# GuoleiSun/VSS-CFFM

Measured on AMD Instinct MI355X. Metric: clips/sec (fwd+bwd) CFFM-B1 480x480 T=4 hot path (CFFA+CFM, decoder_focal depth 2), higher is better.
Workload: dtype f32 in/out, f32 accumulate; MFMA operands: split-bf16 (hi+lo, ~2^-17) in the Linear GEMMs, f16 in QK^T/AV

## Files before the change

vss_cffm_amd/csrc/panel_kernels.h:

```cpp
#pragma once
#include "cffm_common.h"
#include "gemm_kernels.h"
#include "dws_kernels.h"

#define PNL_KC 256
#define PNL_THREADS 512
#define PNL_WAVES 8
__device__ __forceinline__ int pnl_off(int row, int chunk) { return row * PNL_KC + (((chunk ^ row) & 15) << 3) + ((chunk & 16) << 3); }
#define PNL_IMG(MT) (16 * (MT) * PNL_KC)
#define PNL_LDS(MT) (2 * 2 * PNL_IMG(MT) * 2 + 2 * PNL_THREADS * 16)

__device__ __host__ __forceinline__ long pnl_frag_unit(int jt, int ks, int h, int KS) { return ((long)(jt * KS + ks) * 2 + h) * 64; }

__device__ __forceinline__ void pnl_pack_weight(const float* __restrict__ W, int N, int K, bool nn, f32x4* __restrict__ dst, long item) {
    const int lane = (int)(item & 63);
    const long u = item >> 6;
    const int OUT = nn ? K : N, KS = (nn ? N : K) / 32;
    const int ks = (int)(u % KS), jt = (int)(u / KS);
    if (jt * 16 >= OUT) return;
    const int l15 = lane & 15, g = lane >> 4;
    bf16x8 hi, lo;
#pragma unroll
    for (int e = 0; e < 8; ++e) {
        const int o = 16 * jt + l15, c = 32 * ks + 8 * g + e;
        const float x = nn ? W[(long)c * K + o] : W[(long)o * K + c];
        hi[e] = (bf16)x;
        lo[e] = (bf16)(x - (float)hi[e]);
    }
    dst[pnl_frag_unit(jt, ks, 0, KS) + lane] = __builtin_bit_cast(f32x4, hi);
    dst[pnl_frag_unit(jt, ks, 1, KS) + lane] = __builtin_bit_cast(f32x4, lo);
}
__global__ void __launch_bounds__(256) k_pnl_pack_weight(const float* __restrict__ W, int N, int K, int nn, f32x4* __restrict__ dst) {
    const long item = (long)blockIdx.x * 256 + threadIdx.x;
    if (item < (long)N * K / 8) pnl_pack_weight(W, N, K, nn != 0, dst, item);
}

struct PnlPackJobs { const float* w[4]; f32x4* dst[4]; int N[4], K[4]; long end[4]; int n, nn; };
__global__ void __launch_bounds__(256) k_pnl_pack_weights(PnlPackJobs J) {
    long item = (long)blockIdx.x * 256 + threadIdx.x;
    int j = 0;
#pragma unroll
    for (int q = 0; q < 3; ++q)
        if (q + 1 < J.n && item >= J.end[q]) j = q + 1;
    if (j > 0) item -= J.end[j - 1];
    if (item < (long)J.N[j] * J.K[j] / 8) pnl_pack_weight(J.w[j], J.N[j], J.K[j], J.nn != 0, J.dst[j], item);
}

__device__ __forceinline__ void pnl_lds_barrier() {
#ifdef CFFM_EMU
    __syncthreads();
#else
    __builtin_amdgcn_fence(__ATOMIC_RELEASE, "workgroup", "local");
    __builtin_amdgcn_s_barrier();
    __builtin_amdgcn_fence(__ATOMIC_ACQUIRE, "workgroup", "local");
#endif
}

template <int MT>
struct PnlStage { f32x4 v[2 * MT]; };
template <int MT>
__device__ __forceinline__ void pnl_stage_load(PnlStage<MT>& r, buf_t rs, int lda, int m0, int kc0, int tid) {
#pragma unroll
    for (int it = 0; it < 2 * MT; ++it) {
        const int item = tid + PNL_THREADS * it, row = item >> 6, c4 = item & 63;
        r.v[it] = buf_ld16(rs, (uint32_t)((row * lda + 4 * c4) * 4), (uint32_t)(((long)m0 * lda + kc0) * 4));
    }
}
template <int MT, bool PRE>
__device__ __forceinline__ void pnl_stage_store(const PnlStage<MT>& r, bf16* __restrict__ hi, bf16* __restrict__ lo, int tid) {
#pragma unroll
    for (int it = 0; it < 2 * MT; ++it) {
        const int item = tid + PNL_THREADS * it, row = item >> 6, c4 = item & 63;
        bf16x4 h, l;
        if (PRE) unsplit4(r.v[it], h, l);
        else split4(r.v[it], h, l);
        const int o = pnl_off(row, c4 >> 1) + 4 * (c4 & 1);
        *(bf16x4*)(hi + o) = h;
        *(bf16x4*)(lo + o) = l;
    }
}

template <int NT, int D>
struct PnlRing { f32x4 v[D][NT][2]; };

struct PnlStream {
    buf_t rs;
    uint32_t voff;
    int KS;
};
template <int NT, int D>
__device__ __forceinline__ void pnl_ring_load(PnlRing<NT, D>& ring, int slot, const PnlStream& st, int jt, int ks) {
#pragma unroll
    for (int j = 0; j < NT; ++j)
#pragma unroll
        for (int h = 0; h < 2; ++h)
            ring.v[slot][j][h] = buf_ld16(st.rs, st.voff, (uint32_t)(pnl_frag_unit(jt + j, ks, h, st.KS) * 16));
}

__device__ __forceinline__ void pnl_pin_vmem() {
#ifndef CFFM_EMU
    __builtin_amdgcn_sched_barrier(0);
#endif
}
struct PnlNoExtra { __device__ __forceinline__ void operator()(int) const {} };
template <int MT, int NTW, int NT, int D, class Extra = PnlNoExtra, bool LAST = false>
__device__ __forceinline__ void pnl_chunk_mma(f32x4 (&acc)[NTW][MT], PnlRing<NT, D>& ring, const bf16* __restrict__ Ahi,
                                              const bf16* __restrict__ Alo, const PnlStream& st, int jt0, int ks0, int l15, int g,
                                              const PnlStream& nst, int njt0, int nks0, const Extra& extra = Extra()) {
    constexpr int NPASS = NTW / NT, SC = NPASS * 8;
    static_assert(NTW % NT == 0 && SC % D == 0 && D <= SC && D >= 2, "ring depth must divide the steps of a chunk");
    bf16x8 ah[2][MT], al[2][MT];
#pragma unroll
    for (int i = 0; i < MT; ++i) {
        ah[0][i] = *(const bf16x8*)(Ahi + pnl_off(16 * i + l15, g));
        al[0][i] = *(const bf16x8*)(Alo + pnl_off(16 * i + l15, g));
    }
#pragma unroll
    for (int sc = 0; sc < SC; ++sc) {
        const int p = sc / 8, cur = sc & 1;
        const int sn = sc + D - 1, slot_n = sn % D;
        if (sn < SC) pnl_ring_load<NT, D>(ring, slot_n, st, jt0 + (sn / 8) * NT, ks0 + sn % 8);
        else if (!LAST) pnl_ring_load<NT, D>(ring, slot_n, nst, njt0 + ((sn - SC) / 8) * NT, nks0 + (sn - SC) % 8);
        extra(sc);
        pnl_pin_vmem();
        if (sc + 1 < SC) {
            const int k8n = (sc + 1) % 8;
#pragma unroll
            for (int i = 0; i < MT; ++i) {
                ah[cur ^ 1][i] = *(const bf16x8*)(Ahi + pnl_off(16 * i + l15, 4 * k8n + g));
                al[cur ^ 1][i] = *(const bf16x8*)(Alo + pnl_off(16 * i + l15, 4 * k8n + g));
            }
        }
        const int slot = sc % D;
#pragma unroll
        for (int j = 0; j < NT; ++j) {
            const bf16x8 bh = __builtin_bit_cast(bf16x8, ring.v[slot][j][0]), bl = __builtin_bit_cast(bf16x8, ring.v[slot][j][1]);
#pragma unroll
            for (int i = 0; i < MT; ++i) {
                f32x4 c = acc[p * NT + j][i];
                c = mfma16x16x32_bf16(bh, al[cur][i], c);
                c = mfma16x16x32_bf16(bl, ah[cur][i], c);
                c = mfma16x16x32_bf16(bh, ah[cur][i], c);
                acc[p * NT + j][i] = c;
            }
        }
    }
}

template <int MT>
__device__ __forceinline__ void pnl_tfrag_store(const bf16* __restrict__ hi, const bf16* __restrict__ lo, f32x4* __restrict__ dst, int m0, int jt0, int CT,
                                                long R, long R32, int wave, int lane) {
    const int l15 = lane & 15, g = lane >> 4;
    constexpr int NRG = 2 * MT, NOP = (NRG + 3) / 4;
#pragma unroll
    for (int q = 0; q < 32 * NOP / PNL_WAVES; ++q) {
        const int item = wave + PNL_WAVES * q;
        const int u = item / NOP, op = item % NOP, jt = u >> 1, h = u & 1;
        const int rgl = 4 * op + g;
        const bf16* img = h ? lo : hi;
        const int row = 8 * (rgl < NRG ? rgl : 0) + (l15 >> 2), col = 16 * jt + 4 * (l15 & 3);
        const bf16x4 a = lds_tr4_bf16(img + pnl_off(row, col >> 3) + (col & 4));
        const bf16x4 b = lds_tr4_bf16(img + pnl_off(row + 4, col >> 3) + (col & 4));
        const long rg = (long)(m0 >> 3) + rgl, r0 = 8 * rg;
        bf16x8 f;
#pragma unroll
        for (int e = 0; e < 4; ++e) {
            f[e] = r0 + e < R ? a[e] : (bf16)0.f;
            f[4 + e] = r0 + 4 + e < R ? b[e] : (bf16)0.f;
        }
        const bool tail = (NRG % 4 != 0) && rgl >= NRG && (long)m0 + 16 * MT >= R;
        if ((rgl < NRG || tail) && r0 < R32) dst[tfrag_unit(rg >> 2, jt0 + jt, h, CT) + 16 * (int)(rg & 3) + l15] = __builtin_bit_cast(f32x4, f);
    }
}

__device__ __forceinline__ uint32_t pnl_l2_touch(const void* w, long bytes, int tid) {
    const long nlines = bytes >> 7;
    const int nsl = (int)(gridDim.x >> 3) > 0 ? (int)(gridDim.x >> 3) : 1, rank = (int)(blockIdx.x >> 3) % nsl;
    const long per = (nlines + nsl - 1) / nsl, l = rank * per + tid;
    return (tid < per && l < nlines) ? *(const uint32_t*)((const char*)w + (l << 7)) : 0u;
}
template <int MT, int NTW, int NT, int D, bool A_PRE, int EPI>
__global__ void __launch_bounds__(PNL_THREADS) k_panel_gemm(const float* __restrict__ A, int lda, int M, int K, const f32x4* __restrict__ Wf,
                                                            float* __restrict__ C, int ldc, const float* __restrict__ bias,
                                                            float* __restrict__ colrec = nullptr,
                                                            f32x4* __restrict__ a_t = nullptr ) {
    CFFM_DYN_SMEM(smem);
    bf16* img = (bf16*)smem;
    f32x4* csum = (f32x4*)(img + 4 * PNL_IMG(MT));
#define PNL_COLSUM_PUT(c_)                                                                        \
    if (!A_PRE && colrec) {                                                                       \
        f32x4 s_ = sr.v[0];                                                                       \
        _Pragma("unroll") for (int it = 1; it < 2 * MT; ++it) s_ += sr.v[it];                     \
        csum[((c_) & 1) * PNL_THREADS + tid] = s_;                                                \
    }
#define PNL_COLSUM_GET(c_)                                                                        \
    if (!A_PRE && colrec && wave == ((c_) & 7)) {                                                 \
        const f32x4* p_ = csum + ((c_) & 1) * PNL_THREADS + lane;                                 \
        f32x4 t_ = p_[0];                                                                         \
        _Pragma("unroll") for (int w = 1; w < PNL_WAVES; ++w) t_ += p_[64 * w];                   \
        *(f32x4*)(colrec + (long)blockIdx.x * K + (c_) * PNL_KC + 4 * lane) = t_;                 \
    }
    const int tid = threadIdx.x, lane = tid & 63, wave = wave_uniform(tid >> 6), l15 = lane & 15, g = lane >> 4;
    const int m0 = blockIdx.x * 16 * MT;
    const int NCH = K / PNL_KC, KS = K / 32, N = PNL_WAVES * NTW * 16;
    const buf_t rsa = buf_make(A, (uint32_t)((long)M * lda * 4));
    PnlStream st;
    st.rs = buf_make(Wf, (uint32_t)((long)N * K * 4));
    st.voff = lane * 16;
    st.KS = KS;
    const int jt0 = wave * NTW;
    f32x4 acc[NTW][MT];
#pragma unroll
    for (int t = 0; t < NTW; ++t)
#pragma unroll
        for (int i = 0; i < MT; ++i) acc[t][i] = (f32x4){0.f, 0.f, 0.f, 0.f};
    PnlRing<NT, D> ring;
#pragma unroll
    for (int s = 0; s < D - 1; ++s) pnl_ring_load<NT, D>(ring, s, st, jt0 + (s / 8) * NT, s % 8);
    pnl_pin_vmem();
    PnlStage<MT> sr;
    pnl_stage_load<MT>(sr, rsa, lda, m0, 0, tid);
    pnl_stage_store<MT, A_PRE>(sr, img, img + PNL_IMG(MT), tid);
    PNL_COLSUM_PUT(0)
    if (NCH > 1) pnl_stage_load<MT>(sr, rsa, lda, m0, PNL_KC, tid);
    pnl_lds_barrier();
    for (int c = 0; c < NCH; ++c) {
        PNL_COLSUM_GET(c)
        const bf16* hi = img + (c & 1) * 2 * PNL_IMG(MT);
        pnl_chunk_mma<MT, NTW, NT, D>(acc, ring, hi, hi + PNL_IMG(MT), st, jt0, 8 * c, l15, g, st, jt0, 8 * (c + 1));
        if (a_t) pnl_tfrag_store<MT>(hi, hi + PNL_IMG(MT), a_t, m0, 16 * c, K / 16, M, ((long)M + 31) / 32 * 32, wave, lane);
        if (c + 1 < NCH) {
            bf16* nx = img + ((c + 1) & 1) * 2 * PNL_IMG(MT);
            pnl_stage_store<MT, A_PRE>(sr, nx, nx + PNL_IMG(MT), tid);
            PNL_COLSUM_PUT(c + 1)
            if (c + 2 < NCH) pnl_stage_load<MT>(sr, rsa, lda, m0, (c + 2) * PNL_KC, tid);
            pnl_lds_barrier();
        }
    }
#undef PNL_COLSUM_PUT
#undef PNL_COLSUM_GET
    {
        static_assert(EPI == 0, "k_panel_gemm epilogue");
        constexpr int ESZ = 4, NCOL = PNL_WAVES * NTW * 16, ROWB = NCOL * ESZ + 32, UPR = NCOL * ESZ / 16;
        static_assert(16 * MT * ROWB <= PNL_LDS(MT), "panel output does not fit the image buffers");
        char* out = (char*)smem;
        __syncthreads();
#pragma unroll
        for (int t = 0; t < NTW; ++t) {
            const int n = 16 * (jt0 + t) + 4 * g;
            f32x4 bv = (f32x4){0.f, 0.f, 0.f, 0.f};
            if (bias) bv = *(const f32x4*)(bias + n);
#pragma unroll
            for (int i = 0; i < MT; ++i) {
                *(f32x4*)(out + (16 * i + l15) * ROWB + n * ESZ) = acc[t][i] + bv;
            }
        }
        __syncthreads();
        char* dst = (char*)C;
        for (int u = tid; u < 16 * MT * UPR; u += PNL_THREADS) {
            const int r = u / UPR, c = u % UPR;
            if (m0 + r < M) *(f32x4*)(dst + ((long)(m0 + r) * ldc) * ESZ + 16 * c) = *(const f32x4*)(out + r * ROWB + 16 * c);
        }
    }
}

#define QKV3_LDS(MT) (2 * PNL_IMG(MT) * 2)
template <int MT>
__global__ void __launch_bounds__(PNL_THREADS, 4) k_panel_qkv3(const float* __restrict__ xs, int M, const f32x4* __restrict__ Wf,
                                                               const float* __restrict__ bias, h16* __restrict__ qkv16, f32x4* __restrict__ x_t) {
    constexpr int NTW = 2, D = 2, KS = CFFM_C / 32;
    static_assert(CFFM_C == PNL_KC && PNL_WAVES * NTW * 16 == CFFM_C, "one chunk, 256 columns per third");
    CFFM_DYN_SMEM(smem);
    bf16* img = (bf16*)smem;
    const int tid = threadIdx.x, lane = tid & 63, wave = wave_uniform(tid >> 6), l15 = lane & 15, g = lane >> 4;
    const int q = blockIdx.x >> 3, t = q % 3, pan = 8 * (q / 3) + (blockIdx.x & 7);
    if (pan >= (M + 16 * MT - 1) / (16 * MT)) return;
    const int m0 = pan * 16 * MT;
    const buf_t rsa = buf_make(xs, (uint32_t)((long)M * CFFM_C * 4));
    PnlStream st;
    st.rs = buf_make(Wf, (uint32_t)(3 * CFFM_C * CFFM_C * 4));
    st.voff = lane * 16;
    st.KS = KS;
    const int jt0 = 16 * t + wave * NTW;
    f32x4 acc[NTW][MT];
#pragma unroll
    for (int j = 0; j < NTW; ++j)
#pragma unroll
        for (int i = 0; i < MT; ++i) acc[j][i] = (f32x4){0.f, 0.f, 0.f, 0.f};
    PnlRing<2, D> ring;
    pnl_ring_load<2, D>(ring, 0, st, jt0, 0);
    pnl_pin_vmem();
    {
        PnlStage<MT> sr;
        pnl_stage_load<MT>(sr, rsa, CFFM_C, m0, 0, tid);
        pnl_stage_store<MT, true>(sr, img, img + PNL_IMG(MT), tid);
    }
    pnl_lds_barrier();
    pnl_chunk_mma<MT, NTW, 2, D, PnlNoExtra, true>(acc, ring, img, img + PNL_IMG(MT), st, jt0, 0, l15, g, st, jt0, 0);
    if (x_t && t == 0) pnl_tfrag_store<MT>(img, img + PNL_IMG(MT), x_t, m0, 0, CFFM_C / 16, M, ((long)M + 31) / 32 * 32, wave, lane);
    constexpr int ROWB = CFFM_C * 2 + 32, UPR = CFFM_C * 2 / 16;
    static_assert(16 * MT * ROWB <= QKV3_LDS(MT), "panel output does not fit the image");
    char* out = (char*)smem;
    pnl_lds_barrier();
    const float sc = t == 0 ? 0.17677669529663687f : 1.f;
#pragma unroll
    for (int j = 0; j < NTW; ++j) {
        const int nl = 16 * (wave * NTW + j) + 4 * g;
        const f32x4 bv = *(const f32x4*)(bias + CFFM_C * t + nl);
#pragma unroll
        for (int i = 0; i < MT; ++i) {
            typedef h16 h16x4 __attribute__((ext_vector_type(4)));
            h16x4 o;
            for (int e = 0; e < 4; ++e) o[e] = (h16)((acc[j][i][e] + bv[e]) * sc);
            *(h16x4*)(out + (16 * i + l15) * ROWB + nl * 2) = o;
        }
    }
    pnl_lds_barrier();
    char* dst = (char*)qkv16 + CFFM_C * 2 * t;
    for (int u = tid; u < 16 * MT * UPR; u += PNL_THREADS) {
        const int r = u / UPR, c = u % UPR;
        if (m0 + r < M) *(f32x4*)(dst + (long)(m0 + r) * (3 * CFFM_C * 2) + 16 * c) = *(const f32x4*)(out + r * ROWB + 16 * c);
    }
}

__device__ __forceinline__ f32x4 pnl_pack_hl(bf16x4 h, bf16x4 l) {
    const f32x2_t a = __builtin_bit_cast(f32x2_t, h), b = __builtin_bit_cast(f32x2_t, l);
    return (f32x4){a[0], a[1], b[0], b[1]};
}
__device__ __forceinline__ void pnl_img_put(bf16* __restrict__ hi, bf16* __restrict__ lo, int row, int n, bf16x4 h, bf16x4 l) {
    const int o = pnl_off(row, n >> 3) + (n & 4);
    *(bf16x4*)(hi + o) = h;
    *(bf16x4*)(lo + o) = l;
}
__device__ __forceinline__ float pnl_sum_g(float v) {
    v += __shfl_xor(v, 16, 64);
    v += __shfl_xor(v, 32, 64);
    return v;
}
#define PNL_STORE4(p, v) (*(f32x4*)(p) = (v))
#define PNL_FUSED_LDS(MT) (6 * PNL_IMG(MT) * 2 + 2 * PNL_WAVES * 16 * (MT) * 4)

struct MlpFwdArgs {
    const float* ao;
    const float* xt; long xt_bs; int rows_per_batch;
    const f32x4 *wp, *w1, *w2;
    const float *bp, *b1, *b2, *g2, *be2;
    float *x1, *z2s , *mean2, *rstd2, *hraw, *acts , *x2;
    f32x4 *ao_t, *z2_t, *act_t;
    int NP;
};

template <int MT, int D, bool INFER = false>
__global__ void __launch_bounds__(PNL_THREADS) k_mlp_fwd(MlpFwdArgs a) {
    CFFM_DYN_SMEM(smem);
    bf16* P = (bf16*)smem;
    bf16* ACT = P + 2 * PNL_IMG(MT);
    float* red = (float*)(ACT + 4 * PNL_IMG(MT));
    const int tid = threadIdx.x, lane = tid & 63, wave = wave_uniform(tid >> 6), l15 = lane & 15, g = lane >> 4;
    const int m0 = blockIdx.x * 16 * MT, NP = a.NP;
    PnlStream sp, s1, s2;
    sp.rs = buf_make(a.wp, 256u * 256 * 4); sp.voff = lane * 16; sp.KS = 8;
    s1.rs = buf_make(a.w1, 1024u * 256 * 4); s1.voff = lane * 16; s1.KS = 8;
    s2.rs = buf_make(a.w2, 1024u * 256 * 4); s2.voff = lane * 16; s2.KS = 32;
    PnlRing<2, D> ring;
#pragma unroll
    for (int s = 0; s < D - 1; ++s) pnl_ring_load<2, D>(ring, s, sp, 2 * wave, s);
    uint32_t touch = 0;
    pnl_pin_vmem();
    {
        PnlStage<MT> sr;
        pnl_stage_load<MT>(sr, buf_make(a.ao, (uint32_t)((long)NP * 256 * 4)), 256, m0, 0, tid);
        pnl_pin_vmem();
        const uint32_t t0 = pnl_l2_touch(a.w1, 1024L * 256 * 4, tid), t1 = pnl_l2_touch(a.w2, 1024L * 256 * 4, tid);
        pnl_pin_vmem();
        pnl_stage_store<MT, false>(sr, P, P + PNL_IMG(MT), tid);
        touch = t0 ^ t1;
    }
    pnl_lds_barrier();
    const long NP32 = ((long)NP + 31) / 32 * 32;
    if (!INFER && a.ao_t) pnl_tfrag_store<MT>(P, P + PNL_IMG(MT), a.ao_t, m0, 0, 16, NP, NP32, wave, lane);
    const f32x4 z4 = (f32x4){0.f, 0.f, 0.f, 0.f};
    f32x4 acc[2][MT];
#pragma unroll
    for (int t = 0; t < 2; ++t)
#pragma unroll
        for (int i = 0; i < MT; ++i) acc[t][i] = z4;
    pnl_chunk_mma<MT, 2, 2, D>(acc, ring, P, P + PNL_IMG(MT), sp, 2 * wave, 0, l15, g, s1, 2 * wave, 0);
    f32x4 x1v[2][MT];
    bool valid[MT];
    long mrow[MT];
    float s[MT];
#pragma unroll
    for (int i = 0; i < MT; ++i) {
        const long m = m0 + 16 * i + l15;
        valid[i] = m < NP;
        mrow[i] = m;
        s[i] = 0.f;
    }
#pragma unroll
    for (int t = 0; t < 2; ++t) {
        const int n = 32 * wave + 16 * t + 4 * g;
        const f32x4 bv = *(const f32x4*)(a.bp + n);
#pragma unroll
        for (int i = 0; i < MT; ++i) {
            f32x4 r = z4;
            if (valid[i]) {
                const long b = mrow[i] / a.rows_per_batch, rr = mrow[i] % a.rows_per_batch;
                r = *(const f32x4*)(a.xt + b * a.xt_bs + rr * 256 + n);
            }
            const f32x4 v = acc[t][i] + bv + r;
            x1v[t][i] = v;
            if (!INFER && valid[i]) *(f32x4*)(a.x1 + mrow[i] * 256 + n) = v;
            s[i] += (v[0] + v[1]) + (v[2] + v[3]);
        }
    }
#pragma unroll
    for (int i = 0; i < MT; ++i) {
        s[i] = pnl_sum_g(s[i]);
        if (g == 0) red[wave * 16 * MT + 16 * i + l15] = s[i];
    }
    pnl_lds_barrier();
    float mu[MT], rs[MT];
#pragma unroll
    for (int i = 0; i < MT; ++i) {
        float tot = 0.f;
#pragma unroll
        for (int w = 0; w < PNL_WAVES; ++w) tot += red[w * 16 * MT + 16 * i + l15];
        mu[i] = tot * (1.f / 256);
        float q = 0.f;
#pragma unroll
        for (int t = 0; t < 2; ++t) {
            const f32x4 d = x1v[t][i] - mu[i];
            q += (d[0] * d[0] + d[1] * d[1]) + (d[2] * d[2] + d[3] * d[3]);
        }
        q = pnl_sum_g(q);
        if (g == 0) red[(PNL_WAVES + wave) * 16 * MT + 16 * i + l15] = q;
    }
    pnl_lds_barrier();
#pragma unroll
    for (int i = 0; i < MT; ++i) {
        float tot = 0.f;
#pragma unroll
        for (int w = 0; w < PNL_WAVES; ++w) tot += red[(PNL_WAVES + w) * 16 * MT + 16 * i + l15];
        rs[i] = 1.f / sqrtf(tot * (1.f / 256) + CFFM_LN_EPS);
        if (!INFER && wave == 0 && g == 0 && valid[i]) { a.mean2[mrow[i]] = mu[i]; a.rstd2[mrow[i]] = rs[i]; }
    }
#pragma unroll
    for (int t = 0; t < 2; ++t) {
        const int n = 32 * wave + 16 * t + 4 * g;
        const f32x4 gm = *(const f32x4*)(a.g2 + n), be = *(const f32x4*)(a.be2 + n);
#pragma unroll
        for (int i = 0; i < MT; ++i) {
            const f32x4 zv = (x1v[t][i] - mu[i]) * rs[i] * gm + be;
            bf16x4 h, l;
            split4(zv, h, l);
            pnl_img_put(P, P + PNL_IMG(MT), 16 * i + l15, n, h, l);
            if (!INFER && valid[i] && a.z2s) *(f32x4*)(a.z2s + mrow[i] * 256 + n) = pnl_pack_hl(h, l);
        }
    }
    pnl_lds_barrier();
    if (!INFER && a.z2_t) pnl_tfrag_store<MT>(P, P + PNL_IMG(MT), a.z2_t, m0, 0, 16, NP, NP32, wave, lane);
    f32x4 acc2[2][MT];
#pragma unroll
    for (int t = 0; t < 2; ++t)
#pragma unroll
        for (int i = 0; i < MT; ++i) acc2[t][i] = z4;
    for (int c = 0; c < 4; ++c) {
        f32x4 h1[2][MT];
#pragma unroll
        for (int t = 0; t < 2; ++t)
#pragma unroll
            for (int i = 0; i < MT; ++i) h1[t][i] = z4;
        pnl_chunk_mma<MT, 2, 2, D>(h1, ring, P, P + PNL_IMG(MT), s1, 16 * c + 2 * wave, 0, l15, g, s2, 2 * wave, 8 * c);
        bf16* Ah = ACT + (c & 1) * 2 * PNL_IMG(MT);
#pragma unroll
        for (int t = 0; t < 2; ++t) {
            const int nl = 32 * wave + 16 * t + 4 * g, n = 256 * c + nl;
            const f32x4 bv = *(const f32x4*)(a.b1 + n);
#pragma unroll
            for (int i = 0; i < MT; ++i) {
                const f32x4 raw = h1[t][i];
                f32x4 av;
                for (int e = 0; e < 4; ++e) av[e] = gelu_erf(raw[e] + bv[e]);
                bf16x4 h, l;
                split4(av, h, l);
                pnl_img_put(Ah, Ah + PNL_IMG(MT), 16 * i + l15, nl, h, l);
                if (!INFER && valid[i]) {
                    *(f32x4*)(a.hraw + mrow[i] * 1024 + n) = raw;
                    if (a.acts) *(f32x4*)(a.acts + mrow[i] * 1024 + n) = pnl_pack_hl(h, l);
                }
            }
        }
        pnl_lds_barrier();
        if (!INFER && a.act_t) pnl_tfrag_store<MT>(Ah, Ah + PNL_IMG(MT), a.act_t, m0, 16 * c, 64, NP, NP32, wave, lane);
        const int cn = c < 3 ? c + 1 : 0;
        pnl_chunk_mma<MT, 2, 2, D>(acc2, ring, Ah, Ah + PNL_IMG(MT), s2, 2 * wave, 8 * c, l15, g, s1, 16 * cn + 2 * wave, 0);
    }
#pragma unroll
    for (int t = 0; t < 2; ++t) {
        const int n = 32 * wave + 16 * t + 4 * g;
        const f32x4 bv = *(const f32x4*)(a.b2 + n);
#pragma unroll
        for (int i = 0; i < MT; ++i)
            if (valid[i]) *(f32x4*)(a.x2 + mrow[i] * 256 + n) = x1v[t][i] + acc2[t][i] + bv;
    }
    if (a.NP < 0) (INFER ? a.x2 : a.mean2)[tid] = (float)touch;
}

struct MlpBwdArgs {
    const float* dout;
    const float* hraw; const float* b1;
    const float *x1, *mean2, *rstd2, *g2;
    const f32x4 *w2n, *w1n, *wpn;
    float* dhs;
    f32x4 *dout_t, *dh_t, *dx1_t;
    float* dx1;
    float* dao;
    float* rec_b1;
    float* rec_ln;
    int NP;
};

template <int MT, int D>
__global__ void __launch_bounds__(PNL_THREADS) k_mlp_bwd(MlpBwdArgs a) {
    CFFM_DYN_SMEM(smem);
    bf16* P = (bf16*)smem;
    bf16* DH = P + 2 * PNL_IMG(MT);
    float* red = (float*)(DH + 4 * PNL_IMG(MT));
    const int tid = threadIdx.x, lane = tid & 63, wave = wave_uniform(tid >> 6), l15 = lane & 15, g = lane >> 4;
    const int m0 = blockIdx.x * 16 * MT, NP = a.NP;
    PnlStream s2, s1, sp;
    s2.rs = buf_make(a.w2n, 1024u * 256 * 4); s2.voff = lane * 16; s2.KS = 8;
    s1.rs = buf_make(a.w1n, 1024u * 256 * 4); s1.voff = lane * 16; s1.KS = 32;
    sp.rs = buf_make(a.wpn, 256u * 256 * 4); sp.voff = lane * 16; sp.KS = 8;
    PnlRing<2, D> ring;
#pragma unroll
    for (int s = 0; s < D - 1; ++s) pnl_ring_load<2, D>(ring, s, s2, 2 * wave, s);
    uint32_t touch = 0;
    pnl_pin_vmem();
    const buf_t rs_dout = buf_make(a.dout, (uint32_t)((long)NP * 256 * 4));
    {
        PnlStage<MT> sr;
        pnl_stage_load<MT>(sr, rs_dout, 256, m0, 0, tid);
        pnl_pin_vmem();
        const uint32_t t0 = pnl_l2_touch(a.w2n, 1024L * 256 * 4, tid), t1 = pnl_l2_touch(a.w1n, 1024L * 256 * 4, tid), t2 = pnl_l2_touch(a.wpn, 256L * 256 * 4, tid);
        pnl_pin_vmem();
        pnl_stage_store<MT, false>(sr, P, P + PNL_IMG(MT), tid);
        touch = t0 ^ t1 ^ t2;
    }
    pnl_lds_barrier();
    const long NP32 = ((long)NP + 31) / 32 * 32;
    if (a.dout_t) pnl_tfrag_store<MT>(P, P + PNL_IMG(MT), a.dout_t, m0, 0, 16, NP, NP32, wave, lane);
    const f32x4 z4 = (f32x4){0.f, 0.f, 0.f, 0.f};
    bool valid[MT];
    long mrow[MT];
#pragma unroll
    for (int i = 0; i < MT; ++i) {
        const long m = m0 + 16 * i + l15;
        valid[i] = m < NP;
        mrow[i] = m;
    }
    f32x4 dz[2][MT];
#pragma unroll
    for (int t = 0; t < 2; ++t)
#pragma unroll
        for (int i = 0; i < MT; ++i) dz[t][i] = z4;
    for (int c = 0; c < 4; ++c) {
        f32x4 da[2][MT];
#pragma unroll
        for (int t = 0; t < 2; ++t)
#pragma unroll
            for (int i = 0; i < MT; ++i) da[t][i] = z4;
        f32x4 hr[2][MT];
#pragma unroll
        for (int t = 0; t < 2; ++t)
#pragma unroll
            for (int i = 0; i < MT; ++i) hr[t][i] = valid[i] ? *(const f32x4*)(a.hraw + mrow[i] * 1024 + 256 * c + 32 * wave + 16 * t + 4 * g) : z4;
        pnl_pin_vmem();
        pnl_chunk_mma<MT, 2, 2, D>(da, ring, P, P + PNL_IMG(MT), s2, 16 * c + 2 * wave, 0, l15, g, s1, 2 * wave, 8 * c);
        bf16* Ah = DH + (c & 1) * 2 * PNL_IMG(MT);
#pragma unroll
        for (int t = 0; t < 2; ++t) {
            const int nl = 32 * wave + 16 * t + 4 * g, n = 256 * c + nl;
            const f32x4 bv = *(const f32x4*)(a.b1 + n);
            f32x4 cs = z4;
#pragma unroll
            for (int i = 0; i < MT; ++i) {
                f32x4 dh = z4;
                if (valid[i]) {
                    const f32x4 hv = hr[t][i] + bv;
                    for (int e = 0; e < 4; ++e) dh[e] = da[t][i][e] * gelu_erf_grad(hv[e]);
                }
                bf16x4 h, l;
                split4(dh, h, l);
                pnl_img_put(Ah, Ah + PNL_IMG(MT), 16 * i + l15, nl, h, l);
                if (valid[i] && a.dhs) *(f32x4*)(a.dhs + mrow[i] * 1024 + n) = pnl_pack_hl(h, l);
                cs += dh;
            }
            for (int e = 0; e < 4; ++e) cs[e] = row16_sum(cs[e]);
            if (l15 == 0) *(f32x4*)(a.rec_b1 + (long)blockIdx.x * 1024 + n) = cs;
        }
        pnl_lds_barrier();
        if (a.dh_t) pnl_tfrag_store<MT>(Ah, Ah + PNL_IMG(MT), a.dh_t, m0, 16 * c, 64, NP, NP32, wave, lane);
        const bool more = c < 3;
        pnl_chunk_mma<MT, 2, 2, D>(dz, ring, Ah, Ah + PNL_IMG(MT), s1, 2 * wave, 8 * c, l15, g, more ? s2 : sp, more ? 16 * (c + 1) + 2 * wave : 2 * wave, 0);
    }
    f32x4 xh[2][MT], gz[2][MT], dr[2][MT];
    float mu[MT], rs[MT], m1[MT], m2[MT];
#pragma unroll
    for (int i = 0; i < MT; ++i) {
        mu[i] = valid[i] ? a.mean2[mrow[i]] : 0.f;
        rs[i] = valid[i] ? a.rstd2[mrow[i]] : 0.f;
        m1[i] = m2[i] = 0.f;
    }
    f32x4 ag[2], ab[2], ar[2], ax[2];
#pragma unroll
    for (int t = 0; t < 2; ++t) {
        const int n = 32 * wave + 16 * t + 4 * g;
        const f32x4 gm = *(const f32x4*)(a.g2 + n);
        ag[t] = ab[t] = ar[t] = ax[t] = z4;
#pragma unroll
        for (int i = 0; i < MT; ++i) {
            f32x4 xv = z4, dv = z4;
            if (valid[i]) {
                xv = *(const f32x4*)(a.x1 + mrow[i] * 256 + n);
                dv = *(const f32x4*)(a.dout + mrow[i] * 256 + n);
            }
            xh[t][i] = (xv - mu[i]) * rs[i];
            dr[t][i] = dv;
            gz[t][i] = dz[t][i] * gm;
            ag[t] += dz[t][i] * xh[t][i];
            ab[t] += dz[t][i];
            ar[t] += dv;
            const f32x4 p = gz[t][i] * xh[t][i];
            m1[i] += (gz[t][i][0] + gz[t][i][1]) + (gz[t][i][2] + gz[t][i][3]);
            m2[i] += (p[0] + p[1]) + (p[2] + p[3]);
        }
    }
#pragma unroll
    for (int i = 0; i < MT; ++i) {
        m1[i] = pnl_sum_g(m1[i]);
        m2[i] = pnl_sum_g(m2[i]);
        if (g == 0) {
            red[wave * 16 * MT + 16 * i + l15] = m1[i];
            red[(PNL_WAVES + wave) * 16 * MT + 16 * i + l15] = m2[i];
        }
    }
    pnl_lds_barrier();
#pragma unroll
    for (int i = 0; i < MT; ++i) {
        float t1 = 0.f, t2 = 0.f;
#pragma unroll
        for (int w = 0; w < PNL_WAVES; ++w) {
            t1 += red[w * 16 * MT + 16 * i + l15];
            t2 += red[(PNL_WAVES + w) * 16 * MT + 16 * i + l15];
        }
        m1[i] = t1 * (1.f / 256);
        m2[i] = t2 * (1.f / 256);
    }
#pragma unroll
    for (int t = 0; t < 2; ++t) {
        const int n = 32 * wave + 16 * t + 4 * g;
#pragma unroll
        for (int i = 0; i < MT; ++i) {
            const f32x4 dxv = (gz[t][i] - m1[i] - xh[t][i] * m2[i]) * rs[i] + dr[t][i];
            ax[t] += dxv;
            bf16x4 h, l;
            split4(dxv, h, l);
            pnl_img_put(P, P + PNL_IMG(MT), 16 * i + l15, n, h, l);
            if (valid[i]) *(f32x4*)(a.dx1 + mrow[i] * 256 + n) = dxv;
        }
        for (int e = 0; e < 4; ++e) {
            ag[t][e] = row16_sum(ag[t][e]);
            ab[t][e] = row16_sum(ab[t][e]);
            ar[t][e] = row16_sum(ar[t][e]);
            ax[t][e] = row16_sum(ax[t][e]);
        }
        if (l15 == 0) {
            float* rec = a.rec_ln + (long)blockIdx.x * 1024 + n;
            *(f32x4*)(rec) = ag[t];
            *(f32x4*)(rec + 256) = ab[t];
            *(f32x4*)(rec + 512) = ar[t];
            *(f32x4*)(rec + 768) = ax[t];
        }
    }
    pnl_lds_barrier();
    if (a.dx1_t) pnl_tfrag_store<MT>(P, P + PNL_IMG(MT), a.dx1_t, m0, 0, 16, NP, NP32, wave, lane);
    f32x4 dq[2][MT];
#pragma unroll
    for (int t = 0; t < 2; ++t)
#pragma unroll
        for (int i = 0; i < MT; ++i) dq[t][i] = z4;
    pnl_chunk_mma<MT, 2, 2, D>(dq, ring, P, P + PNL_IMG(MT), sp, 2 * wave, 0, l15, g, sp, 2 * wave, 8);
#pragma unroll
    for (int t = 0; t < 2; ++t) {
        const int n = 32 * wave + 16 * t + 4 * g;
#pragma unroll
        for (int i = 0; i < MT; ++i)
            if (valid[i]) *(f32x4*)(a.dao + mrow[i] * 256 + n) = dq[t][i];
    }
    if (a.NP < 0) a.dao[tid] = (float)touch;
}
```

Measured before the change: 2970.

## Prefetch epilogue operands and hraw chunks ahead of MFMA phases in MLP kernels

```diff
diff --git a/vss_cffm_amd/csrc/panel_kernels.h b/vss_cffm_amd/csrc/panel_kernels.h
--- a/vss_cffm_amd/csrc/panel_kernels.h
+++ b/vss_cffm_amd/csrc/panel_kernels.h
@@ -367,9 +367,32 @@
     for (int s = 0; s < D - 1; ++s) pnl_ring_load<2, D>(ring, s, sp, 2 * wave, s);
     uint32_t touch = 0;
     pnl_pin_vmem();
+    const f32x4 z4 = (f32x4){0.f, 0.f, 0.f, 0.f};
+    bool valid[MT];
+    long mrow[MT];
+#pragma unroll
+    for (int i = 0; i < MT; ++i) {
+        const long m = m0 + 16 * i + l15;
+        valid[i] = m < NP;
+        mrow[i] = m;
+    }
+    f32x4 xtv[2][MT], bpv[2];
     {
         PnlStage<MT> sr;
         pnl_stage_load<MT>(sr, buf_make(a.ao, (uint32_t)((long)NP * 256 * 4)), 256, m0, 0, tid);
+#pragma unroll
+        for (int t = 0; t < 2; ++t) {
+            const int n = 32 * wave + 16 * t + 4 * g;
+            bpv[t] = *(const f32x4*)(a.bp + n);
+#pragma unroll
+            for (int i = 0; i < MT; ++i) {
+                xtv[t][i] = z4;
+                if (valid[i]) {
+                    const long b = mrow[i] / a.rows_per_batch, rr = mrow[i] % a.rows_per_batch;
+                    xtv[t][i] = *(const f32x4*)(a.xt + b * a.xt_bs + rr * 256 + n);
+                }
+            }
+        }
         pnl_pin_vmem();
         const uint32_t t0 = pnl_l2_touch(a.w1, 1024L * 256 * 4, tid), t1 = pnl_l2_touch(a.w2, 1024L * 256 * 4, tid);
         pnl_pin_vmem();
@@ -379,7 +402,6 @@
     pnl_lds_barrier();
     const long NP32 = ((long)NP + 31) / 32 * 32;
     if (!INFER && a.ao_t) pnl_tfrag_store<MT>(P, P + PNL_IMG(MT), a.ao_t, m0, 0, 16, NP, NP32, wave, lane);
-    const f32x4 z4 = (f32x4){0.f, 0.f, 0.f, 0.f};
     f32x4 acc[2][MT];
 #pragma unroll
     for (int t = 0; t < 2; ++t)
@@ -387,28 +409,23 @@
         for (int i = 0; i < MT; ++i) acc[t][i] = z4;
     pnl_chunk_mma<MT, 2, 2, D>(acc, ring, P, P + PNL_IMG(MT), sp, 2 * wave, 0, l15, g, s1, 2 * wave, 0);
     f32x4 x1v[2][MT];
-    bool valid[MT];
-    long mrow[MT];
     float s[MT];
 #pragma unroll
-    for (int i = 0; i < MT; ++i) {
-        const long m = m0 + 16 * i + l15;
-        valid[i] = m < NP;
-        mrow[i] = m;
-        s[i] = 0.f;
-    }
+    for (int i = 0; i < MT; ++i) s[i] = 0.f;
+    f32x4 gmv[2], bev[2];
 #pragma unroll
     for (int t = 0; t < 2; ++t) {
         const int n = 32 * wave + 16 * t + 4 * g;
-        const f32x4 bv = *(const f32x4*)(a.bp + n);
+        gmv[t] = *(const f32x4*)(a.g2 + n);
+        bev[t] = *(const f32x4*)(a.be2 + n);
+    }
+    pnl_pin_vmem();
+#pragma unroll
+    for (int t = 0; t < 2; ++t) {
+        const int n = 32 * wave + 16 * t + 4 * g;
 #pragma unroll
         for (int i = 0; i < MT; ++i) {
-            f32x4 r = z4;
-            if (valid[i]) {
-                const long b = mrow[i] / a.rows_per_batch, rr = mrow[i] % a.rows_per_batch;
-                r = *(const f32x4*)(a.xt + b * a.xt_bs + rr * 256 + n);
-            }
-            const f32x4 v = acc[t][i] + bv + r;
+            const f32x4 v = acc[t][i] + bpv[t] + xtv[t][i];
             x1v[t][i] = v;
             if (!INFER && valid[i]) *(f32x4*)(a.x1 + mrow[i] * 256 + n) = v;
             s[i] += (v[0] + v[1]) + (v[2] + v[3]);
@@ -448,7 +465,7 @@
 #pragma unroll
     for (int t = 0; t < 2; ++t) {
         const int n = 32 * wave + 16 * t + 4 * g;
-        const f32x4 gm = *(const f32x4*)(a.g2 + n), be = *(const f32x4*)(a.be2 + n);
+        const f32x4 gm = gmv[t], be = bev[t];
 #pragma unroll
         for (int i = 0; i < MT; ++i) {
             const f32x4 zv = (x1v[t][i] - mu[i]) * rs[i] * gm + be;
@@ -465,18 +482,25 @@
     for (int t = 0; t < 2; ++t)
 #pragma unroll
         for (int i = 0; i < MT; ++i) acc2[t][i] = z4;
+    f32x4 b2v[2];
+#pragma unroll
+    for (int t = 0; t < 2; ++t) b2v[t] = *(const f32x4*)(a.b2 + 32 * wave + 16 * t + 4 * g);
     for (int c = 0; c < 4; ++c) {
         f32x4 h1[2][MT];
 #pragma unroll
         for (int t = 0; t < 2; ++t)
 #pragma unroll
             for (int i = 0; i < MT; ++i) h1[t][i] = z4;
+        f32x4 b1v[2];
+#pragma unroll
+        for (int t = 0; t < 2; ++t) b1v[t] = *(const f32x4*)(a.b1 + 256 * c + 32 * wave + 16 * t + 4 * g);
+        pnl_pin_vmem();
         pnl_chunk_mma<MT, 2, 2, D>(h1, ring, P, P + PNL_IMG(MT), s1, 16 * c + 2 * wave, 0, l15, g, s2, 2 * wave, 8 * c);
         bf16* Ah = ACT + (c & 1) * 2 * PNL_IMG(MT);
 #pragma unroll
         for (int t = 0; t < 2; ++t) {
             const int nl = 32 * wave + 16 * t + 4 * g, n = 256 * c + nl;
-            const f32x4 bv = *(const f32x4*)(a.b1 + n);
+            const f32x4 bv = b1v[t];
 #pragma unroll
             for (int i = 0; i < MT; ++i) {
                 const f32x4 raw = h1[t][i];
@@ -499,7 +523,7 @@
 #pragma unroll
     for (int t = 0; t < 2; ++t) {
         const int n = 32 * wave + 16 * t + 4 * g;
-        const f32x4 bv = *(const f32x4*)(a.b2 + n);
+        const f32x4 bv = b2v[t];
 #pragma unroll
         for (int i = 0; i < MT; ++i)
             if (valid[i]) *(f32x4*)(a.x2 + mrow[i] * 256 + n) = x1v[t][i] + acc2[t][i] + bv;
@@ -539,9 +563,27 @@
     uint32_t touch = 0;
     pnl_pin_vmem();
     const buf_t rs_dout = buf_make(a.dout, (uint32_t)((long)NP * 256 * 4));
+    const f32x4 z4 = (f32x4){0.f, 0.f, 0.f, 0.f};
+    bool valid[MT];
+    long mrow[MT];
+#pragma unroll
+    for (int i = 0; i < MT; ++i) {
+        const long m = m0 + 16 * i + l15;
+        valid[i] = m < NP;
+        mrow[i] = m;
+    }
+    f32x4 hr[2][2][MT];
+    const auto hr_request = [&](int c) {
+#pragma unroll
+        for (int t = 0; t < 2; ++t)
+#pragma unroll
+            for (int i = 0; i < MT; ++i)
+                hr[c & 1][t][i] = valid[i] ? *(const f32x4*)(a.hraw + mrow[i] * 1024 + 256 * c + 32 * wave + 16 * t + 4 * g) : z4;
+    };
     {
         PnlStage<MT> sr;
         pnl_stage_load<MT>(sr, rs_dout, 256, m0, 0, tid);
+        hr_request(0);
         pnl_pin_vmem();
         const uint32_t t0 = pnl_l2_touch(a.w2n, 1024L * 256 * 4, tid), t1 = pnl_l2_touch(a.w1n, 1024L * 256 * 4, tid), t2 = pnl_l2_touch(a.wpn, 256L * 256 * 4, tid);
         pnl_pin_vmem();
@@ -551,44 +593,60 @@
     pnl_lds_barrier();
     const long NP32 = ((long)NP + 31) / 32 * 32;
     if (a.dout_t) pnl_tfrag_store<MT>(P, P + PNL_IMG(MT), a.dout_t, m0, 0, 16, NP, NP32, wave, lane);
-    const f32x4 z4 = (f32x4){0.f, 0.f, 0.f, 0.f};
-    bool valid[MT];
-    long mrow[MT];
-#pragma unroll
-    for (int i = 0; i < MT; ++i) {
-        const long m = m0 + 16 * i + l15;
-        valid[i] = m < NP;
-        mrow[i] = m;
-    }
     f32x4 dz[2][MT];
 #pragma unroll
     for (int t = 0; t < 2; ++t)
 #pragma unroll
         for (int i = 0; i < MT; ++i) dz[t][i] = z4;
+    f32x4 dr[2][MT], gmv[2];
+    float mu[MT], rs[MT];
+#pragma unroll
     for (int c = 0; c < 4; ++c) {
         f32x4 da[2][MT];
 #pragma unroll
         for (int t = 0; t < 2; ++t)
 #pragma unroll
             for (int i = 0; i < MT; ++i) da[t][i] = z4;
-        f32x4 hr[2][MT];
-#pragma unroll
-        for (int t = 0; t < 2; ++t)
-#pragma unroll
-            for (int i = 0; i < MT; ++i) hr[t][i] = valid[i] ? *(const f32x4*)(a.hraw + mrow[i] * 1024 + 256 * c + 32 * wave + 16 * t + 4 * g) : z4;
+        f32x4 b1v[2];
+#pragma unroll
+        for (int t = 0; t < 2; ++t) b1v[t] = *(const f32x4*)(a.b1 + 256 * c + 32 * wave + 16 * t + 4 * g);
         pnl_pin_vmem();
         pnl_chunk_mma<MT, 2, 2, D>(da, ring, P, P + PNL_IMG(MT), s2, 16 * c + 2 * wave, 0, l15, g, s1, 2 * wave, 8 * c);
+        const bool more = c < 3;
+        if (more) {
+            hr_request(c + 1);
+        } else {
+#pragma unroll
+            for (int i = 0; i < MT; ++i) {
+                mu[i] = valid[i] ? a.mean2[mrow[i]] : 0.f;
+                rs[i] = valid[i] ? a.rstd2[mrow[i]] : 0.f;
+            }
+#pragma unroll
+            for (int t = 0; t < 2; ++t) {
+                const int n = 32 * wave + 16 * t + 4 * g;
+                gmv[t] = *(const f32x4*)(a.g2 + n);
+#pragma unroll
+                for (int i = 0; i < MT; ++i) {
+                    hr[(c + 1) & 1][t][i] = dr[t][i] = z4;
+                    if (valid[i]) {
+                        hr[(c + 1) & 1][t][i] = *(const f32x4*)(a.x1 + mrow[i] * 256 + n);
+                        dr[t][i] = *(const f32x4*)(a.dout + mrow[i] * 256 + n);
+                    }
+                }
+            }
+        }
+        pnl_pin_vmem();
         bf16* Ah = DH + (c & 1) * 2 * PNL_IMG(MT);
 #pragma unroll
         for (int t = 0; t < 2; ++t) {
             const int nl = 32 * wave + 16 * t + 4 * g, n = 256 * c + nl;
-            const f32x4 bv = *(const f32x4*)(a.b1 + n);
+            const f32x4 bv = b1v[t];
             f32x4 cs = z4;
 #pragma unroll
             for (int i = 0; i < MT; ++i) {
                 f32x4 dh = z4;
                 if (valid[i]) {
-                    const f32x4 hv = hr[t][i] + bv;
+                    const f32x4 hv = hr[c & 1][t][i] + bv;
                     for (int e = 0; e < 4; ++e) dh[e] = da[t][i][e] * gelu_erf_grad(hv[e]);
                 }
                 bf16x4 h, l;
@@ -602,32 +660,22 @@
         }
         pnl_lds_barrier();
         if (a.dh_t) pnl_tfrag_store<MT>(Ah, Ah + PNL_IMG(MT), a.dh_t, m0, 16 * c, 64, NP, NP32, wave, lane);
-        const bool more = c < 3;
         pnl_chunk_mma<MT, 2, 2, D>(dz, ring, Ah, Ah + PNL_IMG(MT), s1, 2 * wave, 8 * c, l15, g, more ? s2 : sp, more ? 16 * (c + 1) + 2 * wave : 2 * wave, 0);
     }
-    f32x4 xh[2][MT], gz[2][MT], dr[2][MT];
-    float mu[MT], rs[MT], m1[MT], m2[MT];
-#pragma unroll
-    for (int i = 0; i < MT; ++i) {
-        mu[i] = valid[i] ? a.mean2[mrow[i]] : 0.f;
-        rs[i] = valid[i] ? a.rstd2[mrow[i]] : 0.f;
-        m1[i] = m2[i] = 0.f;
-    }
+    f32x4 xh[2][MT], gz[2][MT];
+    float m1[MT], m2[MT];
+#pragma unroll
+    for (int i = 0; i < MT; ++i) m1[i] = m2[i] = 0.f;
     f32x4 ag[2], ab[2], ar[2], ax[2];
 #pragma unroll
     for (int t = 0; t < 2; ++t) {
         const int n = 32 * wave + 16 * t + 4 * g;
-        const f32x4 gm = *(const f32x4*)(a.g2 + n);
+        const f32x4 gm = gmv[t];
         ag[t] = ab[t] = ar[t] = ax[t] = z4;
 #pragma unroll
         for (int i = 0; i < MT; ++i) {
-            f32x4 xv = z4, dv = z4;
-            if (valid[i]) {
-                xv = *(const f32x4*)(a.x1 + mrow[i] * 256 + n);
-                dv = *(const f32x4*)(a.dout + mrow[i] * 256 + n);
-            }
+            const f32x4 xv = hr[0][t][i], dv = dr[t][i];
             xh[t][i] = (xv - mu[i]) * rs[i];
-            dr[t][i] = dv;
             gz[t][i] = dz[t][i] * gm;
             ag[t] += dz[t][i] * xh[t][i];
             ab[t] += dz[t][i];
```

Measured after the change: 3048 (median of 6 runs). +2.6%, better.
